# JuanTarrio/rebvo

Hardware: AMD Instinct MI355X
Metric: frames/sec (DoG+extract+track+depth) 752x480 EuRoC (higher is better)
Workload: dtype f32 scale-space / f64 tracker+EKF

## Files before the change

### rebvo_amd/csrc/api.hip

```cpp

#include <math.h>
#include <stdio.h>
#include <stdlib.h>
#include <string.h>

#include <algorithm>
#include <mutex>

#include "ctx.h"
#include "stage_a_dev.h"

namespace edgehip {

static thread_local std::string g_err;

int wait_pinned_ring(edgehip_ctx *c) {
    const int r = c->frames_seen % 8;
    if (c->ring_valid[r]) EH_CHECK(hipEventSynchronize(c->ev_ring[r]));
    return 0;
}

static int wait_idx_row(edgehip_ctx *c, int slot, const int32_t *pi) {
    if (c->slot_src[slot].idx_row != pi) return 0;
    if (c->a_api_valid[slot]) EH_CHECK(hipEventSynchronize(c->ev_a[slot]));
// ... 405 lines not shown
    }
    EH_TRY(dmalloc(c, &c->div_lut, kDivLutMax, al->dev));
    EH_TRY(dmalloc(c, &c->pinv, 3 * 49, al->dev, 0));
    EH_TRY(dmalloc(c, &c->seq, B, al->dev, 0));
    EH_TRY(dmalloc(c, &c->seqa, B, al->dev, 0));
    EH_TRY(dmalloc(c, &c->tresh_slot, S * B, al->dev, 0));
    c->fc_rows = std::max<int>(nslots, kRefRing);
    c->fc_index = 0;
    EH_TRY(dmalloc(c, &c->framecount, (size_t)c->fc_rows * B, al->dev, 0));
    EH_TRY(dmalloc(c, &c->kn_slot, S * B, al->dev, 0));
    EH_TRY(dmalloc(c, &c->retuned_slot, S * B, al->dev, 0));
    c->band_rows = detect_band_rows(p.w, p.plane_fit_size);
    c->nbands = (p.h - 2 * p.plane_fit_size + c->band_rows - 1) / c->band_rows;
    {
        const int npx = c->band_rows * p.w, nchunk = (npx + 63) / 64, cpw = (nchunk + kDetWaves - 1) / kDetWaves;
        c->band_cap = cpw * 64;
    }
    const size_t nstrips = (size_t)c->nbands * kDetWaves;
    EH_TRY(dmalloc(c, &c->band_cnt, B * nstrips, al->dev, 0));
    EH_TRY(dmalloc(c, &c->band_off, B * (nstrips + 1), al->dev, 0));
    {
        char *bs;
        EH_TRY(dmalloc(c, &bs, B * nstrips * c->band_cap * 20, al->dev));
        c->band_stage = bs;
    }
    EH_TRY(dmalloc(c, &c->histo, B * 256, al->dev, 0));
    c->nblk_tvr = (int)((CAP + kTvrBlock - 1) / kTvrBlock);
    EH_TRY(dmalloc(c, &c->P0, B * 3 * CAP, al->dev, 0));
    EH_TRY(dmalloc(c, &c->resid, (size_t)kResidBufs * B * CAP, al->dev, 0));
    EH_TRY(dmalloc(c, &c->resid_carry, (size_t)kResidBufs * B * c->nblk_tvr, al->dev, 0));
    EH_TRY(dmalloc(c, &c->partials, 2 * B * c->nblk_tvr * kNumSums, al->dev, 0));
    EH_TRY(dmalloc(c, &c->block_last, 2 * B * c->nblk_tvr, al->dev, 0));
    EH_TRY(dmalloc(c, &c->bin_cnt, B * 256, al->dev, 0));
    {
        const size_t ntiles = (size_t)((p.w + 63) / 64) * ((p.h + 63) / 64);
        EH_TRY(dmalloc(c, &c->bins, B * ntiles * CAP, al->dev));
    }
    c->field_radius = p.search_range;
    c->field_mode = EH_EXP_ENV("EDGEHIP_FIELD_MODE", 0);
    c->no_grec = getenv("EDGEHIP_NO_GREC") && atoi(getenv("EDGEHIP_NO_GREC")) != 0;
    c->level_mode = getenv("EDGEHIP_LEVEL_MODE") ? atoi(getenv("EDGEHIP_LEVEL_MODE")) : 0;
    c->fwd_mode = EH_EXP_ENV("EDGEHIP_FWD_MODE", 0);
    c->fused_min_batch = fused_min_env;
    c->fused_undist = EH_EXP_ENV("EDGEHIP_FUSED_UNDIST", 0) != 0;
    c->tvr_rw2 = EH_EXP_ENV("EDGEHIP_TVR_RW2", 0);
    c->dual_init = getenv("EDGEHIP_DUAL_INIT") ? atoi(getenv("EDGEHIP_DUAL_INIT")) : 1;
    c->persist_lm_max = EH_EXP_ENV("EDGEHIP_PERSIST_LM", 0);
    EH_TRY(dmalloc(c, &c->sync_cnt, B, al->dev, 0));
    EH_TRY(dmalloc(c, &c->fwd_key, B * CAP, al->dev, 0));
    EH_TRY(dmalloc(c, &c->fwd_win, B * CAP, al->dev, 0xFF));
    EH_TRY(dmalloc(c, &c->rs_tmp, B * 2 * CAP, al->dev, 0));
    c->fuse_match = !(getenv("EDGEHIP_FUSE_MATCH") && atoi(getenv("EDGEHIP_FUSE_MATCH")) == 0);
    if (c->fuse_match) {
        EH_TRY(dmalloc(c, &c->rot_pm, S * B * CAP, al->dev, 0)); EH_TRY(dmalloc(c, &c->rot_mm, S * B * CAP, al->dev, 0));
        EH_TRY(dmalloc(c, &c->rot_rho, S * B * CAP, al->dev, 0)); EH_TRY(dmalloc(c, &c->rot_srho, S * B * CAP, al->dev, 0));
    }
    EH_TRY(dmalloc(c, &c->rot_buf, B * 9, al->dev, 0));
    EH_TRY(dmalloc(c, &c->nav_dev, B, al->dev, 0));
    EH_TRY(dmalloc(c, &c->idx_dev, B, al->dev, 0));
    c->slot_src.assign(S, edgehip_ctx::SlotSrc());
    c->stereo_cnt = nullptr;
    if (p.stereo_available) EH_TRY(dmalloc(c, &c->stereo_cnt, B, al->dev, 0));
    c->nav_log = nullptr;
    c->nav_log_len = 0;

    {
        const size_t al256 = 256;
        auto up = [&](size_t x) { return (x + al256 - 1) / al256 * al256; };
        const bool stereo = p.stereo_available != 0;
        const size_t per = up(CAP * 4) * 8  +
                           up(CAP * 8) * 6  + up(CAP * 8) * 7  + up(CAP * 32) + up(CAP * 16)  +
                           (stereo ? up(CAP * 4) + 2 * up(CAP * 8) : 0);
        char *arena;
        EH_TRY(dmalloc(c, &arena, per * S * B, al->dev, 0));
        c->kl_arena = arena;
        c->kl.resize(S * B);
        for (size_t sb = 0; sb < S * B; sb++) {
            char *q = arena + sb * per;
            KlSoA &k = c->kl[sb];
            auto take = [&](size_t bytes) { char *r = q; q += up(bytes); return r; };
            k.p_inx = (int32_t *)take(CAP * 4);
            k.m_m = (float2 *)take(CAP * 8); k.u_m = (float2 *)take(CAP * 8); k.c_p = (float2 *)take(CAP * 8);
            k.p_m = (float2 *)take(CAP * 8); k.p_m_0 = (float2 *)take(CAP * 8); k.m_m0 = (float2 *)take(CAP * 8);
            k.n_m = (float *)take(CAP * 4);
            k.rho = (double *)take(CAP * 8); k.s_rho = (double *)take(CAP * 8); k.rho_nr = (double *)take(CAP * 8);
            k.s_rho_nr = (double *)take(CAP * 8); k.rho0 = (double *)take(CAP * 8); k.s_rho0 = (double *)take(CAP * 8);
            k.n_m0 = (double *)take(CAP * 8);
            k.m_id = (int32_t *)take(CAP * 4); k.m_id_f = (int32_t *)take(CAP * 4); k.m_id_kf = (int32_t *)take(CAP * 4);
            k.m_num = (int32_t *)take(CAP * 4); k.p_id = (int32_t *)take(CAP * 4); k.n_id = (int32_t *)take(CAP * 4);
            k.rec = (MatchRec *)take(CAP * 32);
            k.grec = (float4 *)take(CAP * 16);
            k.stereo_m_id = nullptr; k.stereo_rho = nullptr; k.stereo_s_rho = nullptr;
            if (stereo) {
                k.stereo_m_id = (int32_t *)take(CAP * 4);
                k.stereo_rho = (double *)take(CAP * 8); k.stereo_s_rho = (double *)take(CAP * 8);
            }
        }
        c->slot_cam.assign(S, edgehip_ctx::SlotCam{pl.ppx, pl.ppy, pl.zfm});
        EH_TRY(dmalloc(c, &c->kl_dev, S * B, al->dev));
        EH_CHECK(hipMemcpyAsync(c->kl_dev, c->kl.data(), sizeof(KlSoA) * S * B, hipMemcpyHostToDevice, c->stream));
    }
    {
        std::vector<float> lut(kDivLutMax, 0.f);
        for (int k = 1; k < kDivLutMax; k++) lut[k] = (float)(1.0 / (double)(float)k);
        EH_CHECK(hipMemcpyAsync(c->div_lut, lut.data(), sizeof(float) * kDivLutMax, hipMemcpyHostToDevice, c->stream));
        double pinv[3 * 49] = {0};
        plane_fit_pinv(p.plane_fit_size, pinv);
        if (p.plane_fit_size == 2)
// ... 1006 lines not shown
```

### rebvo_amd/csrc/ctx.h

```cpp
#pragma once
#include <hip/hip_runtime.h>
#include <stdint.h>
#include <string.h>
#include <string>
#include <map>
#include <vector>
#include <mutex>
#include <atomic>

#include "edgehip.h"
#include "export_ring.h"

namespace edgehip {

constexpr int kMaxBoxes = 3;
constexpr int kBandRows = 12;
constexpr int kDetWaves = 16;
constexpr int kDivLutMax = 256;
constexpr int kTvrThreads = 256;
constexpr int kTvrPasses = 1;
constexpr int kTvrBlock = kTvrThreads * kTvrPasses;
constexpr int kNumSums = 28;
constexpr int kRefRing = 8;
constexpr int kResidBufs = 3;

__host__ __device__ inline uint64_t resid_carry_bits() { return 0x7FF8C0DEC0DEC0DEull; }

struct __attribute__((aligned(16))) MatchRec {
    float c_px, c_py, u_mx, u_my, m_mx, m_my, n_m, pad;
};

struct KlSoA {
    int32_t *p_inx;
    float2 *m_m, *u_m, *c_p, *p_m, *p_m_0, *m_m0;
    float *n_m;
    double *rho, *s_rho, *rho_nr, *s_rho_nr, *rho0, *s_rho0, *n_m0;
    int32_t *m_id, *m_id_f, *m_id_kf, *m_num, *p_id, *n_id;
    MatchRec *rec;
    float4 *grec;
    int32_t *stereo_m_id;
    double *stereo_rho, *stereo_s_rho;
};

struct SeqDev {
    edgehip_seq_state pub;
    int32_t kn_new;
    int32_t band_trunc;
    float nm_max, nm_min;
    double tresh_used;
    double X[6], Xnew[6], Xt[6], h[6];
    double JtJ[36], JtF[6], JtJnew[36], JtFnew[6];
    double F, Fnew, F0, Ft, F0t, u, v, ut, vt, gain;
    int32_t eff_steps, eff_steps_t, res_cur, res_new, res_t, lm_phase;
    int32_t kn_old, pad1;
    double s_rho_min_eval;
    double Rt[9], Vt[3], RM[4];
    int32_t nmatch_tmp, kf_tmp;
    double zX[6], zXnew[6], zh[6];
    double zJtJ[36], zJtF[6], zJtJnew[36], zJtFnew[6];
    double zF, zFnew, zF0, zu, zv, zgain;
    double zRt[9], zVt[3], zRM[4];
    int32_t z_eff_steps, z_pad;
    double mv_V[3], mv_Vnew[3], mv_h[3], mv_JtJ[9], mv_JtF[3], mv_JtJnew[9], mv_JtFnew[3], mv_RVel[9];
    double mv_F, mv_Fnew, mv_u, mv_v, mv_s_rho_min;
    float mv_min_mod; int32_t mv_pad;
    int32_t skip_match, skip_map;
    double t_cur;
    double V_track[3], W_track[3], PV_track[9], PW_track[9];
};

struct SeqA {
    double tresh;
    double tresh_used;
    int32_t l_kl_num;
    int32_t kn_new;
    int32_t band_trunc, pad0;
    float nm_max, nm_min;
    float retuned, pad1;
};

struct DevicePlan {
    int w, h, n, cap, nseq, nslots;
    int ftx;
// ... 271 lines not shown
    edgehip::KlSoA *kl_dev;
    edgehip::SeqDev *seq;
    edgehip::SeqA *seqa;
    double *tresh_slot;
    uint32_t *framecount;
    int fc_rows;
    int fc_index;
    int32_t *kn_slot;
    float *retuned_slot;
    int32_t *band_cnt;
    int32_t *band_off;
    void *band_stage;
    int nbands, band_cap;
    int band_rows;
    int32_t *histo;
    double *P0;
    double *resid;
    double *resid_carry;
    double *partials;
    double *block_last;
    bool use_graph;
    std::map<int, hipGraphExec_t> frame_graphs;
    struct StereoRig {
        bool enabled = false;
        int slot_pair = -1;
        double t[3], R[9], max_radius;
    } rig;
    int ring_slots;
    struct SlotSrc { const uint8_t *base = nullptr; std::vector<int32_t> host_idx; bool grey8 = false;
                     const int32_t *idx_row = nullptr; int idx_ring = 0; };
    uint8_t *grey8 = nullptr;
    uint8_t *pinned_grey8 = nullptr;
    std::vector<SlotSrc> slot_src;
    struct SlotCam { float ppx, ppy; double zfm; };
    std::vector<SlotCam> slot_cam;
    int field_radius;
    int field_mode;
    int level_mode;
    int fused_min_batch;
    double pinv_host[3 * 49];
    int32_t *bin_cnt;
    int32_t *bins;
    int nblk_tvr;
    bool fused_undist;
    int tvr_rw2;
    bool tracker_f32 = false;
    int dual_init;
    int persist_lm_max;
    unsigned *sync_cnt;
    unsigned long long *fwd_key;
    int32_t *fwd_win;
    int fwd_mode = 0;
    bool fuse_match = true;
    float2 *rot_pm = nullptr, *rot_mm = nullptr;
    double *rot_rho = nullptr, *rot_srho = nullptr;
    bool rot_pending[4] = {false, false, false, false};
    bool fwd_fill[4] = {false, false, false, false};
    bool fwd_cleared = false;
    bool fwd_keys_posted = false;
    bool fwd_key_in_tvr = false;
    double *rs_tmp;
    double *rot_buf;
    const double *t_src = nullptr;
    edgehip_keyline *aos_dev = nullptr;
    edgehip_keyline *aos_host = nullptr;
    int32_t *aos_req_dev = nullptr, *aos_req_host = nullptr;
    int aos_requests = 0;
    edgehip::ExportRing kl_ring;
    edgehip::ExportRing ros_ring;
    edgehip_nav *nav_dev;
    edgehip_nav *nav_log;
    edgehip_nav_imu *nav_imu_log = nullptr;
    int nav_log_len;
    int32_t *stereo_log = nullptr;
    hipStream_t stream_log = nullptr;
    hipEvent_t ev_log = nullptr;
    hipEvent_t ev_log_ring[8] = {};
    std::mutex log_mu;
    std::atomic<long long> frames_logged{0};
    long long log_first = 0, log_last = -1;
    int32_t *idx_dev;
    int32_t *stereo_cnt;
    uint8_t *pinned_rgb;
    size_t pinned_rgb_bytes;
    edgehip::SeqDev *pinned_seq;
    edgehip::SeqA *pinned_seqa;
    double *pinned_out;
    double *pinned_t;
    int32_t *pinned_idx;
    edgehip_nav *pinned_nav;
    edgehip::Profiler *prof;
    bool imu_enabled = false, imu_pending = false;
    bool imu_pinned_ok = false;
    edgehip_imu_params imu_params;
    edgehip_kf_request *kf_req_dev = nullptr;
    edgehip_kf_result *kf_res_dev = nullptr;
    void *imu_track = nullptr;
    void *imu_filter = nullptr;
    void *imu_snap = nullptr;
    hipStream_t stream_imu = nullptr;
    hipEvent_t ev_imu_snap[2], ev_imu_post[2];
    hipEvent_t ev_imu_mid[2];
    bool imu_post_valid[2] = {false, false};
    edgehip_imu_integrated *imu_in_dev = nullptr;
    edgehip_nav_imu *nav_imu_dev = nullptr;
    edgehip_imu_integrated *pinned_imu = nullptr;
    edgehip_nav_imu *pinned_nav_imu = nullptr;
    struct DepthFill;
// ... 163 lines not shown
```

### rebvo_amd/csrc/stage_c.hip

```cpp

#include <math.h>
#include <string.h>

#include <vector>

#include "ctx.h"
#include "wave_reduce.h"

namespace edgehip {

constexpr double kRhoMax = 20.0, kRhoMin = 1e-3, kRhoInit = 1.0;

__global__ __launch_bounds__(256) void k_fwd_key(const KlSoA *kl_old, const int32_t *__restrict__ kn_old,
                                                 const int32_t *__restrict__ kn_new, unsigned long long *__restrict__ key,
                                                 int cap) {
    const int seq = blockIdx.z, i = blockIdx.x * 256 + threadIdx.x;
    if (i >= kn_old[seq]) return;
    const int f = kl_old[seq].m_id_f[i];
    if (f < 0 || f >= kn_new[seq]) return;
    atomicMax(&key[(size_t)seq * cap + f], ord_bits(kl_old[seq].rho[i]));
}
__device__ inline void so3_exp_c(const double w[3], double R[9]);
__device__ inline void rot_from_state(SeqDev *sq, double *__restrict__ Rbuf_seq);
__device__ inline void glue_after_tracking(SeqDev *sq);
__global__ __launch_bounds__(256) void k_fwd_win(const KlSoA *kl_old, const int32_t *__restrict__ kn_old,
                                                 const int32_t *__restrict__ kn_new, const unsigned long long *__restrict__ key,
                                                 int32_t *__restrict__ win, int cap, SeqDev *tail_seqs, double *__restrict__ tail_Rbuf) {
    const int seq = blockIdx.z, i = blockIdx.x * 256 + threadIdx.x;
    if (tail_seqs && i == 0) {
        rot_from_state(tail_seqs + seq, tail_Rbuf + (size_t)seq * 9);
        glue_after_tracking(tail_seqs + seq);
    }
    if (i >= kn_old[seq]) return;
    const int f = kl_old[seq].m_id_f[i];
    if (f < 0 || f >= kn_new[seq]) return;
    if (key[(size_t)seq * cap + f] == ord_bits(kl_old[seq].rho[i])) atomicMax(&win[(size_t)seq * cap + f], i);
}
template <bool FILL>
__global__ __launch_bounds__(256) void k_fwd_apply(const KlSoA *kl_old, const KlSoA *kl_new, const int32_t *__restrict__ kn_new,
                                                   const int32_t *__restrict__ win, SeqDev *seqs, int cap) {
    const int seq = blockIdx.z, f = blockIdx.x * 256 + threadIdx.x;
    int hit = 0;
    if (f < kn_new[seq]) {
        const int i = win[(size_t)seq * cap + f];
        const KlSoA &o = kl_old[seq], &n = kl_new[seq];
        if (i >= 0 || FILL) {
            double rho = kRhoInit, s_rho = kRhoMax, rho_nr = kRhoInit, s_rho_nr = kRhoMax;
            int32_t m_num = -1, m_id_kf = -1;
            float2 pm = make_float2(0.f, 0.f), mm = make_float2(0.f, 0.f);
            float nm = 0.f;
            if (i >= 0) {
                rho = o.rho[i]; s_rho = o.s_rho[i]; rho_nr = o.rho_nr[i]; s_rho_nr = o.s_rho_nr[i];
                m_num = o.m_num[i]; m_id_kf = o.m_id_kf[i];
                pm = o.p_m[i]; mm = o.m_m[i];
                nm = o.n_m[i];
            } else {
                pm = n.p_m[f];
            }
            n.rho[f] = rho;
            n.s_rho[f] = s_rho;
            n.rho_nr[f] = rho_nr;
            n.s_rho_nr[f] = s_rho_nr;
            n.m_num[f] = m_num + 1;
            n.m_id[f] = i;
            n.p_m_0[f] = pm;
            n.m_m0[f] = mm;
            n.n_m0[f] = (double)nm;
            n.m_id_kf[f] = m_id_kf;
            hit = i >= 0;
        }
    }
    const int cnt = __popcll(__ballot(hit));
    if ((threadIdx.x & 63) == 0 && cnt) atomicAdd(&seqs[seq].pub.klm_fwd, cnt);
}

__device__ inline void so3_exp_c(const double w[3], double R[9]);

struct RotOut {
    float2 *p_m, *m_m;
    double *rho, *s_rho;
};
struct WinArgs {
    const int32_t *kn_new;
    const unsigned long long *key;
    int32_t *win;
    SeqDev *seqs;
    double *Rbuf;
};
template <bool OUT, bool WIN>
__global__ __launch_bounds__(256) void k_rotate(const KlSoA *kls, const int32_t *__restrict__ kns, const double *__restrict__ Rin,
                                                double zf, RotOut out, int cap, WinArgs wa) {
    const int seq = blockIdx.z, i = blockIdx.x * 256 + threadIdx.x;
    __shared__ double s_R[9];
    if (WIN) {
        if (blockIdx.x * 256 >= kns[seq] && blockIdx.x != 0) return;
        if (threadIdx.x == 0) {
            SeqDev *sq = wa.seqs + seq;
            double R0[9];
            so3_exp_c(sq->pub.W, R0);
            for (int q = 0; q < 9; q++) s_R[q] = R0[q];
            if (blockIdx.x == 0) {
                for (int q = 0; q < 9; q++) wa.Rbuf[(size_t)seq * 9 + q] = R0[q];
                for (int a = 0; a < 3; a++)
                    for (int b = 0; b < 3; b++) sq->pub.R[a * 3 + b] = R0[b * 3 + a];
                glue_after_tracking(sq);
            }
        }
        __syncthreads();
    }
    if (i >= kns[seq]) return;
    double Rw[9];
    if (WIN) {
#pragma unroll
        for (int q = 0; q < 9; q++) {
            const double v = s_R[q];
            const unsigned lo = __builtin_amdgcn_readfirstlane((unsigned)__double2loint(v)), hi = __builtin_amdgcn_readfirstlane((unsigned)__double2hiint(v));
            Rw[q] = __hiloint2double((int)hi, (int)lo);
        }
    }
    const double *R = WIN ? Rw : Rin + (size_t)seq * 9;
    const KlSoA &k = kls[seq];
    const float2 pm = k.p_m[i];
    const float2 m = k.m_m[i];
    const double rho = k.rho[i], s_rho = k.s_rho[i];
    const double v0 = (double)pm.x / zf, v1 = (double)pm.y / zf, v2 = 1;
    double q0 = 0, q1 = 0, q2 = 0;
    q0 += R[0] * v0; q0 += R[1] * v1; q0 += R[2] * v2;
    q1 += R[3] * v0; q1 += R[4] * v1; q1 += R[5] * v2;
    q2 += R[6] * v0; q2 += R[7] * v1; q2 += R[8] * v2;
    const double m0 = (double)m.x, m1 = (double)m.y;
    double r0 = 0, r1 = 0;
    r0 += R[0] * m0; r0 += R[1] * m1; r0 += R[2] * 0.0;
    r1 += R[3] * m0; r1 += R[4] * m1; r1 += R[5] * 0.0;
    const float2 mr = make_float2((float)r0, (float)r1);
    if (WIN) {
        const int f = k.m_id_f[i];
        if (f >= 0 && f < wa.kn_new[seq] && wa.key[(size_t)seq * cap + f] == ord_bits(rho)) atomicMax(&wa.win[(size_t)seq * cap + f], i);
    }
    if (OUT) {
        const size_t o = (size_t)seq * cap + i;
        const bool turn = fabs(q2) > 0;
#if EDGEHIP_NT_ROT
        st_stream(out.p_m + o, turn ? make_float2((float)(q0 / q2 * zf), (float)(q1 / q2 * zf)) : pm);
        st_stream(out.rho + o, turn ? rho / q2 : rho);
        st_stream(out.s_rho + o, turn ? s_rho / q2 : s_rho);
        st_stream(out.m_m + o, mr);
#else
        out.p_m[o] = turn ? make_float2((float)(q0 / q2 * zf), (float)(q1 / q2 * zf)) : pm;
        out.rho[o] = turn ? rho / q2 : rho;
        out.s_rho[o] = turn ? s_rho / q2 : s_rho;
        out.m_m[o] = mr;
#endif
        return;
    }
    if (fabs(q2) > 0) {
        k.p_m[i] = make_float2((float)(q0 / q2 * zf), (float)(q1 / q2 * zf));
        k.rho[i] = rho / q2;
        k.s_rho[i] = s_rho / q2;
    }
    k.m_m[i] = mr;
}

__global__ __launch_bounds__(256) void k_rot_materialize(const KlSoA *kls, const int32_t *__restrict__ kns, RotOut src, int cap) {
    const int seq = blockIdx.z, i = blockIdx.x * 256 + threadIdx.x;
    if (i >= kns[seq]) return;
    const KlSoA &k = kls[seq];
    const size_t o = (size_t)seq * cap + i;
    const float2 pm = src.p_m[o], mm = src.m_m[o];
    const double rho = src.rho[o], s_rho = src.s_rho[o];
    k.p_m[i] = pm; k.m_m[i] = mm; k.rho[i] = rho; k.s_rho[i] = s_rho;
}
static RotOut rot_of(edgehip_ctx *c, int slot) {
    const size_t off = (size_t)slot * c->plan.nseq * c->plan.cap;
    RotOut r;
    r.p_m = c->rot_pm + off; r.m_m = c->rot_mm + off; r.rho = c->rot_rho + off; r.s_rho = c->rot_srho + off;
    return r;
}
int rot_materialize_enqueue(edgehip_ctx *c, int slot) {
    if (slot < 0 || slot >= c->plan.nslots || !c->rot_pending[slot]) return 0;
    const DevicePlan &pl = c->plan;
    hipLaunchKernelGGL(k_rot_materialize, dim3((pl.cap + 255) / 256, 1, pl.nseq), dim3(256), 0, c->stream, kldev(c, slot),
                       c->kn_slot + (size_t)slot * pl.nseq, rot_of(c, slot), pl.cap);
    EH_LAUNCH_CHECK();
    c->rot_pending[slot] = false;
    return 0;
}

__global__ __launch_bounds__(256) void k_rec_refresh(const KlSoA *kls, const int32_t *__restrict__ kns) {
    const int seq = blockIdx.z, i = blockIdx.x * 256 + threadIdx.x;
    if (i >= kns[seq]) return;
    const KlSoA &k = kls[seq];
    const float2 cp = k.c_p[i], um = k.u_m[i], m = k.m_m[i];
    const float nm = k.n_m[i];
    MatchRec rec;
    rec.c_px = cp.x; rec.c_py = cp.y; rec.u_mx = um.x; rec.u_my = um.y;
    rec.m_mx = m.x; rec.m_my = m.y; rec.n_m = nm; rec.pad = 0.f;
    k.rec[i] = rec;
}
int rec_refresh_enqueue(edgehip_ctx *c, int slot) {
    if (int e = rot_materialize_enqueue(c, slot)) return e;
    if (!c->rec_stale[slot]) return 0;
    const DevicePlan &pl = c->plan;
    hipLaunchKernelGGL(k_rec_refresh, dim3((pl.cap + 255) / 256, 1, pl.nseq), dim3(256), 0, c->stream, kldev(c, slot),
                       c->kn_slot + (size_t)slot * pl.nseq);
    EH_LAUNCH_CHECK();
    c->rec_stale[slot] = false;
    return 0;
}

#ifdef EDGEHIP_EXPERIMENTS
__global__ __launch_bounds__(256) void k_fwd_apply_rotate(const KlSoA *kl_old, const KlSoA *kl_new, const int32_t *__restrict__ kn_old,
                                                          const int32_t *__restrict__ kn_new, const int32_t *__restrict__ win,
                                                          SeqDev *seqs, const double *__restrict__ Rin, double zf, int cap) {
    const int seq = blockIdx.z, i = blockIdx.x * 256 + threadIdx.x;
    int hit = 0;
    if (i < kn_old[seq]) {
        const KlSoA &o = kl_old[seq];
        const int f = o.m_id_f[i];
        const float2 pm = o.p_m[i];
        const float2 m = o.m_m[i];
        const double rho = o.rho[i], s_rho = o.s_rho[i];
        if (f >= 0 && f < kn_new[seq] && win[(size_t)seq * cap + f] == i) {
            const KlSoA &n = kl_new[seq];
            const double rho_nr = o.rho_nr[i], s_rho_nr = o.s_rho_nr[i];
            const int32_t m_num = o.m_num[i], m_id_kf = o.m_id_kf[i];
            const float nm = o.n_m[i];
            n.rho[f] = rho;
            n.s_rho[f] = s_rho;
// ... 53 lines not shown
    r[0] = (M[7] - M[5]) / 2;
    r[1] = (M[2] - M[6]) / 2;
    r[2] = (M[3] - M[1]) / 2;
    const double sin_angle_abs = sqrt(r[0] * r[0] + r[1] * r[1] + r[2] * r[2]);
    if (cos_angle > M_SQRT1_2) {
        if (sin_angle_abs > 0) {
            const double s = asin(sin_angle_abs) / sin_angle_abs;
            r[0] *= s; r[1] *= s; r[2] *= s;
        }
    } else if (cos_angle > -M_SQRT1_2) {
        const double s = acos(cos_angle) / sin_angle_abs;
        r[0] *= s; r[1] *= s; r[2] *= s;
    } else {
        const double angle = M_PI - asin(sin_angle_abs);
        const double d0 = M[0] - cos_angle, d1 = M[4] - cos_angle, d2 = M[8] - cos_angle;
        double r2[3];
        if (d0 * d0 > d1 * d1 && d0 * d0 > d2 * d2) { r2[0] = d0; r2[1] = (M[3] + M[1]) / 2; r2[2] = (M[2] + M[6]) / 2; }
        else if (d1 * d1 > d2 * d2) { r2[0] = (M[3] + M[1]) / 2; r2[1] = d1; r2[2] = (M[7] + M[5]) / 2; }
        else { r2[0] = (M[2] + M[6]) / 2; r2[1] = (M[7] + M[5]) / 2; r2[2] = d2; }
        if (r2[0] * r[0] + r2[1] * r[1] + r2[2] * r[2] < 0) { r2[0] = -r2[0]; r2[1] = -r2[1]; r2[2] = -r2[2]; }
        const double nn = sqrt(r2[0] * r2[0] + r2[1] * r2[1] + r2[2] * r2[2]);
        for (int i = 0; i < 3; i++) r[i] = angle * (r2[i] / nn);
    }
}

__device__ inline void rot_from_state(SeqDev *sq, double *__restrict__ Rbuf_seq) {
    double R0[9];
    so3_exp_c(sq->pub.W, R0);
    for (int i = 0; i < 9; i++) Rbuf_seq[i] = R0[i];
    for (int i = 0; i < 3; i++)
        for (int j = 0; j < 3; j++) sq->pub.R[i * 3 + j] = R0[j * 3 + i];
}
__global__ void k_rot_from_state(SeqDev *seqs, double *__restrict__ Rbuf, int nseq) {
    const int seq = blockIdx.x * blockDim.x + threadIdx.x;
    if (seq >= nseq) return;
    rot_from_state(seqs + seq, Rbuf + (size_t)seq * 9);
}

struct DirArgs {
    const KlSoA *kl_new, *kl_old;
    const int32_t *kn_new;
    const int32_t *mask_old;
    SeqDev *seq;
    int w, h;
    size_t n;
    double zfm, min_thr_mod, cang_min_edge, max_radius, loc_unc;
    float ppx, ppy;
    int stereo_mode;
    const int32_t *win;
    RotOut rot;
    int cap;
};

#ifndef EDGEHIP_NT_ROT
#define EDGEHIP_NT_ROT 1
#endif
#ifndef EDGEHIP_NT_EKF
#define EDGEHIP_NT_EKF 1
#endif
#ifndef EDGEHIP_NT_DIRECTED
#define EDGEHIP_NT_DIRECTED 1
#endif
template <bool FUSED, bool FILL>
__device__ __forceinline__ void directed_body(const DirArgs &a) {
    const int seq = blockIdx.z, ik = blockIdx.x * (int)blockDim.x + threadIdx.x;
    SeqDev *sq = a.seq + seq;
    const bool searching = !sq->skip_match;
    if (!FUSED && !searching) return;
    __shared__ double s_v[3], s_rv[9], s_br[9];
    if (threadIdx.x == 0 && searching) {
        const double *BR = sq->pub.R, *V = sq->pub.V, *P = sq->pub.P_V;
        for (int i = 0; i < 9; i++) s_br[i] = BR[i];
        for (int i = 0; i < 3; i++) {
            double d = 0;
            for (int j = 0; j < 3; j++) d += BR[i * 3 + j] * V[j];
            s_v[i] = d;
        }
        double T[9];
        for (int i = 0; i < 3; i++)
            for (int j = 0; j < 3; j++) {
                double d = 0;
                for (int k = 0; k < 3; k++) d += BR[i * 3 + k] * P[k * 3 + j];
                T[i * 3 + j] = d;
            }
        for (int i = 0; i < 3; i++)
            for (int j = 0; j < 3; j++) {
                double d = 0;
                for (int k = 0; k < 3; k++) d += T[i * 3 + k] * BR[j * 3 + k];
                s_rv[i * 3 + j] = d;
            }
    }
    __syncthreads();
    int matched = 0, kfm = 0, fwd = 0;
    if (ik < a.kn_new[seq]) {
        const KlSoA &kn = a.kl_new[seq], &ko = a.kl_old[seq];
        const int32_t *mask = a.mask_old + (size_t)seq * a.n;
        const size_t ro = (size_t)seq * a.cap;
        const float2 kpm = ldg(kn.p_m, ik);
        const float2 kmm = ldg(kn.m_m, ik);
        const float knm = ldg(kn.n_m, ik);
        int iw = -1;
        double krho, ksrho;
        if (FUSED) {
            iw = a.win[ro + ik];
            fwd = iw >= 0;
            if (iw >= 0) { krho = ldg(ko.rho, iw); ksrho = ldg(ko.s_rho, iw); }
            else if (FILL) { krho = kRhoInit; ksrho = kRhoMax; }
            else { krho = ldg(kn.rho, ik); ksrho = ldg(kn.s_rho, ik); }
        } else {
            krho = ldg(kn.rho, ik); ksrho = ldg(kn.s_rho, ik);
        }
        int found = -1;
        if (searching) {
        const double zf = a.zfm;
        double p3[3];
        for (int i = 0; i < 3; i++) {
            double d = 0;
            d += s_br[i * 3 + 0] * (double)kpm.x;
// ... 47 lines not shown
            dq_rho = 0;
            t_steps = (int)dq_max;
        }
        const double norm_m = (double)knm;
        constexpr int DM_CH = 2;
        const double Tmax = (double)(a.w + a.h) + fabs((double)pi0x) + fabs((double)pi0y) + 4.0;
        int seg0[2] = {0, 0}, seg1[2] = {t_steps, 0};
        int nseg = 1;
        if (t_steps > 256 && fabs(dq_rho) < 1e15 && Tmax < 1e15) {
            const double n0 = fmax(0.0, floor(dq_rho - Tmax) - 2.0), n1 = fmin((double)t_steps, ceil(fmin(dq_rho + Tmax, dq_rho - dq_min)) + 2.0);
            const double p0 = fmax(0.0, floor(-Tmax - dq_rho - 1.0) - 2.0), p1 = fmin((double)t_steps, ceil(fmin(Tmax - dq_rho - 1.0, dq_max - dq_rho - 1.0)) + 2.0);
            const bool hn = n1 > n0, hp = p1 > p0;
            nseg = 0;
            if (hn && hp && !(n1 < p0 || p1 < n0)) {
                seg0[0] = (int)fmin(n0, p0); seg1[0] = (int)fmax(n1, p1); nseg = 1;
            } else {
                if (hn) { seg0[nseg] = (int)n0; seg1[nseg] = (int)n1; nseg++; }
                if (hp) { seg0[nseg] = (int)p0; seg1[nseg] = (int)p1; nseg++; }
                if (nseg == 2 && seg0[1] < seg0[0]) {
                    const int s0 = seg0[0], s1 = seg1[0];
                    seg0[0] = seg0[1]; seg1[0] = seg1[1]; seg0[1] = s0; seg1[1] = s1;
                }
            }
        }
        for (int sg = 0; sg < nseg && found < 0; sg++) {
        double tn = dq_rho - (double)seg0[sg], tp = (dq_rho + 1) + (double)seg0[sg];
        const int t_end = seg1[sg];
        for (int t0i = seg0[sg]; t0i < t_end && found < 0; t0i += DM_CH) {
            double tv[DM_CH][2];
            int jm[DM_CH][2];
#pragma unroll
            for (int c = 0; c < DM_CH; c++) {
                tv[c][0] = tn; tv[c][1] = tp;
                tn -= 1; tp += 1;
#pragma unroll
                for (int dir = 0; dir < 2; dir++) {
                    const double t = tv[c][dir];
                    jm[c][dir] = -1;
                    if (t0i + c >= t_end) continue;
                    if (dir ? t > dq_max : t < dq_min) continue;
                    const float fx = (float)(t_x * t + (double)pi0x), fy = (float)(t_y * t + (double)pi0y);
                    const int xi = round_half_away_i(fx), yi = round_half_away_i(fy);
                    if (xi >= a.w || yi >= a.h || xi < 0 || yi < 0) continue;
                    jm[c][dir] = mask[__umul24((unsigned)yi, (unsigned)a.w) + (unsigned)xi];
                }
            }
#pragma unroll
            for (int c = 0; c < DM_CH; c++) {
#pragma unroll
                for (int dir = 0; dir < 2; dir++) {
                    const int j = jm[c][dir];
                    if (j < 0 || found >= 0) continue;
                    const double t = tv[c][dir];
                    const float2 omm = FUSED ? ldg(a.rot.m_m, ro + j) : ldg(ko.m_m, j);
                    const double norm_m0 = (double)ldg(ko.n_m, j);
                    const double cang = div_mid((double)(omm.x * kmm.x + omm.y * kmm.y), norm_m0 * norm_m);
                    if (cang < a.cang_min_edge || fabs(norm_m0 / norm_m - 1) > a.min_thr_mod) continue;
                    const double s_rho = FUSED ? ldg(a.rot.s_rho, ro + j) : ldg(ko.s_rho, j), rho = FUSED ? ldg(a.rot.rho, ro + j) : ldg(ko.rho, j);
                    const double v_rho_dr = (a.loc_unc * a.loc_unc + s_rho * s_rho * norm_t * norm_t + sigma2_t * rho * rho);
                    const double dd = t - norm_t * rho;
                    if (dd * dd > v_rho_dr) continue;
                    found = j;
                }
            }
        }
        }
        }
        if (FUSED) {
            const int src = found >= 0 ? found : iw;
            if (src >= 0 || FILL) {
                double rho = kRhoInit, s_rho = kRhoMax, rho_nr = kRhoInit, s_rho_nr = kRhoMax;
                int32_t m_num = -1, m_id_kf = -1;
                float2 pm, mm = make_float2(0.f, 0.f);
                float nm = 0.f;
                if (src < 0) {
                    pm = ldg(kn.p_m, ik);
                } else {
                    const bool turned = found >= 0;
                    rho = turned ? ldg(a.rot.rho, ro + src) : ldg(ko.rho, src);
                    s_rho = turned ? ldg(a.rot.s_rho, ro + src) : ldg(ko.s_rho, src);
                    pm = turned ? ldg(a.rot.p_m, ro + src) : ldg(ko.p_m, src);
                    mm = turned ? ldg(a.rot.m_m, ro + src) : ldg(ko.m_m, src);
                    rho_nr = ldg(ko.rho_nr, src); s_rho_nr = ldg(ko.s_rho_nr, src);
                    m_num = ldg(ko.m_num, src); m_id_kf = ldg(ko.m_id_kf, src);
                    nm = ldg(ko.n_m, src);
                }
#if EDGEHIP_NT_DIRECTED
                stg_stream(kn.rho, ik, rho);
                stg_stream(kn.s_rho, ik, s_rho);
                stg_stream(kn.rho_nr, ik, rho_nr);
                stg_stream(kn.s_rho_nr, ik, s_rho_nr);
                stg_stream(kn.m_num, ik, m_num + 1);
                stg_stream(kn.m_id, ik, src);
                stg_stream(kn.p_m_0, ik, pm);
                stg_stream(kn.m_m0, ik, mm);
                stg_stream(kn.n_m0, ik, (double)nm);
                stg_stream(kn.m_id_kf, ik, m_id_kf);
#else
                stg(kn.rho, ik, rho);
                stg(kn.s_rho, ik, s_rho);
                stg(kn.rho_nr, ik, rho_nr);
                stg(kn.s_rho_nr, ik, s_rho_nr);
                stg(kn.m_num, ik, m_num + 1);
                stg(kn.m_id, ik, src);
                stg(kn.p_m_0, ik, pm);
                stg(kn.m_m0, ik, mm);
                stg(kn.n_m0, ik, (double)nm);
                stg(kn.m_id_kf, ik, m_id_kf);
#endif
                matched = found >= 0;
                kfm = matched && m_id_kf >= 0;
            }
        } else if (found >= 0) {
            const int j = found;
            const double c_rho = a.stereo_mode ? ldg(ko.rho0, j) : ldg(ko.rho, j), c_srho = a.stereo_mode ? ldg(ko.s_rho0, j) : ldg(ko.s_rho, j);
            double c_rho_nr = 0, c_srho_nr = 0;
            if (!a.stereo_mode) { c_rho_nr = ldg(ko.rho_nr, j); c_srho_nr = ldg(ko.s_rho_nr, j); }
            const int32_t c_mnum = ldg(ko.m_num, j), mk = ldg(ko.m_id_kf, j);
            const float2 c_pm = ldg(ko.p_m, j), c_mm = ldg(ko.m_m, j);
            const float c_nm = ldg(ko.n_m, j);
            stg(kn.rho, ik, c_rho);
            stg(kn.s_rho, ik, c_srho);
            if (!a.stereo_mode) {
                stg(kn.rho_nr, ik, c_rho_nr);
                stg(kn.s_rho_nr, ik, c_srho_nr);
            }
            stg(kn.m_id, ik, j);
            stg(kn.m_num, ik, c_mnum + 1);
            stg(kn.p_m_0, ik, c_pm);
            stg(kn.m_m0, ik, c_mm);
            stg(kn.n_m0, ik, (double)c_nm);
            stg(kn.m_id_kf, ik, mk);
            matched = 1;
            kfm = mk >= 0;
        }
    }
    const int c1 = __popcll(__ballot(matched)), c2 = __popcll(__ballot(kfm)), c3 = FUSED ? __popcll(__ballot(fwd)) : 0;
    if ((threadIdx.x & 63) == 0) {
// ... 496 lines not shown
        if (!c->fwd_cleared) EH_CHECK(hipMemsetAsync(c->fwd_win, 0xFF, sizeof(int32_t) * B * pl.cap, c->stream));
        c->fwd_cleared = false;
        hipLaunchKernelGGL(k_fwd_win, g, b, 0, c->stream, kldev(c, slot_old), kno, knn, c->fwd_key, c->fwd_win, pl.cap,
                           (SeqDev *)nullptr, (double *)nullptr);
        hipLaunchKernelGGL(k_rot_from_state, dim3((pl.nseq + 63) / 64), dim3(64), 0, c->stream, c->seq, c->rot_buf, pl.nseq);
        EH_LAUNCH_CHECK();
    }
    ProfScope ps(c, PROF_C_ROTATE);
    hipLaunchKernelGGL(k_fwd_apply_rotate, g, b, 0, c->stream, kldev(c, slot_old), kldev(c, slot_new), kno, knn, c->fwd_win, c->seq,
                       c->rot_buf, pl.zfm, pl.cap);
    EH_LAUNCH_CHECK();
    return 0;
}
#endif

static inline bool frame_matches_in_one_pass(const edgehip_ctx *c, int slot_pair) {
    return c->fuse_match && c->fwd_mode == 0 && slot_pair < 0 && !c->p.stereo_available;
}

static int forward_rotate_one_pass_enqueue(edgehip_ctx *c, int slot_old, int slot_new) {
    if (int e = rot_materialize_enqueue(c, slot_old)) return e;
    const DevicePlan &pl = c->plan;
    const size_t B = pl.nseq;
    const bool cleared = c->fwd_cleared;
    c->fwd_cleared = false;
    if (!cleared) EH_CHECK(hipMemsetAsync(c->fwd_win, 0xFF, sizeof(int32_t) * B * pl.cap, c->stream));
    c->grec_ok[slot_old] = false;
    c->rec_stale[slot_old] = true;
    ProfScope ps(c, PROF_C_ROTATE);
    WinArgs wa;
    wa.kn_new = c->kn_slot + slot_new * B; wa.key = c->fwd_key; wa.win = c->fwd_win; wa.seqs = c->seq; wa.Rbuf = c->rot_buf;
    hipLaunchKernelGGL((k_rotate<true, true>), dim3((pl.cap + 255) / 256, 1, pl.nseq), dim3(256), 0, c->stream, kldev(c, slot_old),
                       c->kn_slot + slot_old * B, (const double *)nullptr, pl.zfm, rot_of(c, slot_old), pl.cap, wa);
    EH_LAUNCH_CHECK();
    c->rot_pending[slot_old] = true;
    return 0;
}

int rotate_enqueue(edgehip_ctx *c, int slot, const double *R_host, bool R_in_buf) {
    if (int e = rot_materialize_enqueue(c, slot)) return e;
    c->grec_ok[slot] = false;
    c->rec_stale[slot] = true;
    ProfScope ps(c, PROF_C_ROTATE);
    const DevicePlan &pl = c->plan;
    double *Rbuf = c->rot_buf;
    if (R_host) {
        EH_CHECK(hipStreamSynchronize(c->stream));
        memcpy(c->pinned_out, R_host, sizeof(double) * 9 * pl.nseq);
        EH_CHECK(hipMemcpyAsync(Rbuf, c->pinned_out, sizeof(double) * 9 * pl.nseq, hipMemcpyHostToDevice, c->stream));
    } else if (!R_in_buf) {
        hipLaunchKernelGGL(k_rot_from_state, dim3((pl.nseq + 63) / 64), dim3(64), 0, c->stream, c->seq, Rbuf, pl.nseq);
    }
    hipLaunchKernelGGL((k_rotate<false, false>), dim3((pl.cap + 255) / 256, 1, pl.nseq), dim3(256), 0, c->stream, kldev(c, slot),
                       c->kn_slot + (size_t)slot * pl.nseq, Rbuf, pl.zfm, RotOut{nullptr, nullptr, nullptr, nullptr}, pl.cap, WinArgs{});
    EH_LAUNCH_CHECK();
    return 0;
}

struct StereoArgs {
    const KlSoA *kl, *kl_pair;
    const int32_t *kn;
    const int32_t *mask_pair;
    int32_t *nmatch;
    int w, h;
    size_t n;
    double t[3], R[9];
    double zfm0, zfm1;
    float pp1x, pp1y;
    double min_thr_mod, cang_min_edge, max_radius, loc_unc, loc_unc_model;
    const SeqDev *seqs;
};

__global__ __launch_bounds__(256) void k_stereo_match(StereoArgs a) {
    const int seq = blockIdx.z, i = blockIdx.x * 256 + threadIdx.x;
    if (a.seqs && a.seqs[seq].skip_map) return;
    int matched = 0;
    if (i < a.kn[seq]) {
        const KlSoA &k = a.kl[seq], &kp = a.kl_pair[seq];
        const int32_t *mask = a.mask_pair + (size_t)seq * a.n;
        const float2 pm = k.p_m[i], mm = k.m_m[i];
        const float nm = k.n_m[i];
        const double rho = k.rho[i], s_rho = k.s_rho[i];
        const double lo = rho - s_rho, hi = rho + s_rho;
        const double min_rho = lo < 1e-3 ? 1e-3 : lo, max_rho = 20.0 < hi ? 20.0 : hi;
        double q1[2][3];
#pragma unroll
        for (int e = 0; e < 2; e++) {
            const double r = e ? max_rho : min_rho;
            const double p0[3] = {(double)pm.x / r / a.zfm0, (double)pm.y / r / a.zfm0, 1.0 / r};
            double p1[3];
#pragma unroll
            for (int c = 0; c < 3; c++) {
                double d = 0;
                d += a.R[c * 3 + 0] * p0[0]; d += a.R[c * 3 + 1] * p0[1]; d += a.R[c * 3 + 2] * p0[2];
                p1[c] = d + a.t[c];
            }
            q1[e][0] = p1[0] / p1[2] * a.zfm1; q1[e][1] = p1[1] / p1[2] * a.zfm1; q1[e][2] = 1 / p1[2];
        }
        const double dqx = q1[1][0] - q1[0][0], dqy = q1[1][1] - q1[0][1];
        const double pi0x = q1[0][0] + (double)a.pp1x, pi0y = q1[0][1] + (double)a.pp1y;
        double norm_t = sqrt(dqx * dqx + dqy * dqy);
        double t_x, t_y, dq_min, dq_max;
        if (norm_t > 1e-6) {
            t_x = dqx / norm_t;
            t_y = dqy / norm_t;
            dq_min = -a.loc_unc;
            dq_max = fmin(a.max_radius, norm_t + a.loc_unc);
// ... 47 lines not shown
            const double mul = (double)(-u.x) * (zf1 * qh1[0] - qx * qh1[2]) - uy * (zf1 * qh1[1] - qy * qh1[2]);
            double srho = mul / div;
            const double den = qh1[2] + a.t[2] * srho;
            const double df = ux * zf1 * (a.t[0] * den - a.t[2] * (qh1[0] + a.t[0] * srho)) / (den * den) +
                              uy * zf1 * (a.t[1] * den - a.t[2] * (qh1[1] + a.t[1] * srho)) / (den * den);
            double I_rho = (df / a.loc_unc_model) * (df / a.loc_unc_model);
            if (srho != srho || df != df) { srho = 1; I_rho = 1e-10; }
            double ss = 1 / sqrt(I_rho);
            if (srho < 0) { ss = 1e3; srho = 1.0; match = -1; }
            k.stereo_rho[i] = srho;
            k.stereo_s_rho[i] = ss;
        }
        k.stereo_m_id[i] = match;
        matched = match >= 0;
    }
    const int c1 = __popcll(__ballot(matched));
    if ((threadIdx.x & 63) == 0 && c1) atomicAdd(&a.nmatch[seq], c1);
}

__global__ __launch_bounds__(256) void k_fuse_stereo(const KlSoA *kls, const int32_t *__restrict__ kns, SeqDev *seqs) {
    const int seq = blockIdx.z, i = blockIdx.x * 256 + threadIdx.x;
    if (seqs) {
        if (seqs[seq].skip_map) return;
        if (i == 0) seqs[seq].pub.Kp = 1;
    }
    if (i >= kns[seq]) return;
    const KlSoA &k = kls[seq];
    const double r0 = k.rho[i], s0 = k.s_rho[i];
    k.rho0[i] = r0;
    k.s_rho0[i] = s0;
    if (k.stereo_m_id[i] < 0) return;
    const double sr = k.stereo_rho[i], ss = k.stereo_s_rho[i];
    const double s = sqrt(1.0 / (1.0 / (s0 * s0) + 1.0 / (ss * ss)));
    k.s_rho[i] = s;
    k.rho[i] = (r0 / (s0 * s0) + sr / (ss * ss)) * (s * s);
}

int directed_enqueue(edgehip_ctx *c, int slot_new, int slot_old, bool fused) {
    ProfScope ps(c, PROF_C_DIRECTED);
    const DevicePlan &pl = c->plan;
    if (!fused) { if (int e = rot_materialize_enqueue(c, slot_old)) return e; }
    DirArgs a;
    a.kl_new = kldev(c, slot_new); a.kl_old = kldev(c, slot_old);
    a.kn_new = c->kn_slot + (size_t)slot_new * pl.nseq;
    a.mask_old = maskof(c, slot_old);
    a.seq = c->seq; a.w = pl.w; a.h = pl.h; a.n = pl.n; a.zfm = pl.zfm;
    a.min_thr_mod = c->p.match_thresh_module;
    a.cang_min_edge = cos(c->p.match_thresh_angle * M_PI / 180.0);
    a.max_radius = (double)c->p.search_range;
    a.loc_unc = c->p.loc_unc_match;
    a.ppx = pl.ppx; a.ppy = pl.ppy;
    a.stereo_mode = c->p.stereo_available != 0;
    a.win = c->fwd_win; a.cap = pl.cap;
    a.rot = fused ? rot_of(c, slot_old) : RotOut{nullptr, nullptr, nullptr, nullptr};
#ifndef EDGEHIP_DIRECTED_BLOCK
#define EDGEHIP_DIRECTED_BLOCK 128
#endif
    constexpr int kDirBlock = EDGEHIP_DIRECTED_BLOCK;
    const dim3 g((pl.cap + kDirBlock - 1) / kDirBlock, 1, pl.nseq), b(kDirBlock);
    if (fused) {
        if (c->fwd_fill[slot_new]) hipLaunchKernelGGL(k_directed_fused<true>, g, b, 0, c->stream, a);
        else hipLaunchKernelGGL(k_directed_fused<false>, g, b, 0, c->stream, a);
        c->fwd_fill[slot_new] = false;
    } else {
        hipLaunchKernelGGL(k_directed, g, b, 0, c->stream, a);
    }
    EH_LAUNCH_CHECK();
    return 0;
}

int regekf_enqueue(edgehip_ctx *c, int slot, int do_reg, int do_ekf, bool frame_glue) {
    ProfScope ps(c, PROF_C_REGEKF);
    const DevicePlan &pl = c->plan;
    dim3 g((pl.cap + 255) / 256, 1, pl.nseq), b(256);
    const int32_t *kn = c->kn_slot + (size_t)slot * pl.nseq;
    hipLaunchKernelGGL(k_regularize, g, b, 0, c->stream, kldev(c, slot), kn, c->rs_tmp, c->seq, pl.cap,
                       c->p.regularize_thresh, do_reg, frame_glue ? c->p.global_match_threshold : -1);
    hipLaunchKernelGGL(k_ekf, g, b, 0, c->stream, kldev(c, slot), kn, c->rs_tmp, c->seq, pl.cap, pl.zfm, c->p.reshape_q_abs,
                       c->p.loc_unc, do_ekf);
    EH_LAUNCH_CHECK();
    return 0;
}

int rescale_enqueue(edgehip_ctx *c, int slot, bool frame_ends) {
    ProfScope ps(c, PROF_C_RESCALE);
    const DevicePlan &pl = c->plan;
    FrameEndArgs fe = {};
    if (frame_ends) {
        fe.nav = c->nav_dev;
        fe.kn_new = c->kn_slot + (size_t)slot * pl.nseq;
        const int slot_t = c->rig.enabled && c->rig.slot_pair >= 0 ? c->rig.slot_pair : slot;
        fe.tresh_new = c->tresh_slot + (size_t)slot_t * pl.nseq;
        fe.retuned_new = c->retuned_slot + (size_t)slot * pl.nseq;
        fe.nav_log = c->nav_log; fe.nav_log_len = c->nav_log_len; fe.nseq = pl.nseq; fe.have_pair = 1;
    }
    if (!c->lds_optin_rescale) {
        EH_CHECK(hipFuncSetAttribute((const void *)&k_rescale<512, 12, 4>, hipFuncAttributeMaxDynamicSharedMemorySize, 4 * 4 * 1024 * (int)sizeof(double)));
        c->lds_optin_rescale = true;
    }
    hipLaunchKernelGGL((k_rescale<512, 12, 4>), dim3(pl.nseq), dim3(512), 4 * 4 * 1024 * sizeof(double), c->stream, kldev(c, slot),
                       c->kn_slot + (size_t)slot * pl.nseq, c->seq, kRhoMax, 1u, c->p.do_rescaling > 0, fe);
    EH_LAUNCH_CHECK();
    return 0;
}

static int rotate_buf_enqueue(edgehip_ctx *c, int slot) {
    if (int e = rot_materialize_enqueue(c, slot)) return e;
    c->grec_ok[slot] = false;
    c->rec_stale[slot] = true;
    ProfScope ps(c, PROF_C_ROTATE);
    const DevicePlan &pl = c->plan;
    hipLaunchKernelGGL((k_rotate<false, false>), dim3((pl.cap + 255) / 256, 1, pl.nseq), dim3(256), 0, c->stream, kldev(c, slot),
                       c->kn_slot + (size_t)slot * pl.nseq, c->rot_buf, pl.zfm, RotOut{nullptr, nullptr, nullptr, nullptr}, pl.cap, WinArgs{});
    EH_LAUNCH_CHECK();
    return 0;
}
static int ext_rotvel_enqueue(edgehip_ctx *c, int slot) {
    const DevicePlan &pl = c->plan;
    const int B = pl.nseq, nblk = (pl.cap + 255) / 256;
    if (nblk > c->nblk_tvr) { set_error("ext_rot_vel: partial table too small"); return EDGEHIP_ERR_STATE; }
    hipLaunchKernelGGL(k_ext_rotvel, dim3(nblk, 1, B), dim3(256), 0, c->stream, kldev(c, slot), c->kn_slot + (size_t)slot * B,
                       (const double *)nullptr, c->seq, c->partials, c->nblk_tvr, pl.zfm, c->p.loc_unc, c->p.reweight_distance);
    EH_LAUNCH_CHECK();
    return 0;
}

static int glue(edgehip_ctx *c, int mode, int slot_new, int have_pair) {
    const DevicePlan &pl = c->plan;
    const int slot_t = c->rig.enabled && c->rig.slot_pair >= 0 ? c->rig.slot_pair : slot_new;
    hipLaunchKernelGGL(k_frame_glue, dim3((pl.nseq + 63) / 64), dim3(64), 0, c->stream, c->seq, c->t_src, c->nav_dev,
                       c->kn_slot + (size_t)slot_new * pl.nseq, c->tresh_slot + (size_t)slot_t * pl.nseq,
                       c->retuned_slot + (size_t)slot_new * pl.nseq, pl.nseq, mode, c->p.config_fps, c->p.global_match_threshold,
                       have_pair, c->nav_log, c->nav_log_len, c->stereo_cnt, c->rig.enabled ? c->stereo_log : nullptr);
    EH_LAUNCH_CHECK();
    return 0;
}

}

using namespace edgehip;

extern "C" {

static int chk2(edgehip_ctx *c, int a, int b) {
    if (!c || a < 0 || b < 0 || a >= c->plan.nslots || b >= c->plan.nslots) { set_error("slot out of range"); return EDGEHIP_ERR_ARG; }
    if (int e = rot_materialize_enqueue(c, a)) return e;
    return rot_materialize_enqueue(c, b);
}

int edgehip_forward_match(edgehip_ctx *c, int slot_old, int slot_new) {
    EH_ENTER(c);
    if (int e = chk2(c, slot_old, slot_new)) return e;
    return forward_match_enqueue(c, slot_old, slot_new);
}
int edgehip_rotate_keylines(edgehip_ctx *c, int slot, const double *R) {
    EH_ENTER(c);
    if (int e = chk2(c, slot, slot)) return e;
    return rotate_enqueue(c, slot, R);
}
int edgehip_directed_matching(edgehip_ctx *c, int slot_new, int slot_old) {
    EH_ENTER(c);
    if (int e = chk2(c, slot_new, slot_old)) return e;
    return directed_enqueue(c, slot_new, slot_old);
}
int edgehip_match_one_pass(edgehip_ctx *c, int slot_new, int slot_old, int fill) {
    EH_ENTER(c);
// ... 404 lines not shown
```

Measured before the change: 135,500.

## Pack rotated keyline fields into a 32-byte record for the fused matcher

Replaces the separate rotated-buffer arrays for m_m, rho and s_rho with one 32-byte RotRec per keyline that also carries n_m. The rotate kernel writes it with vector nontemporal stores, and the fused directed matcher reads it with two vector loads. The goal is fewer scattered memory transactions on the random-access match candidates. It also adds an XCD-contiguous block remapping for the fused directed kernel, which is off by default.

```diff
diff --git a/rebvo_amd/csrc/api.hip b/rebvo_amd/csrc/api.hip
--- a/rebvo_amd/csrc/api.hip
+++ b/rebvo_amd/csrc/api.hip
@@ -481,8 +481,7 @@
     EH_TRY(dmalloc(c, &c->rs_tmp, B * 2 * CAP, al->dev, 0));
     c->fuse_match = !(getenv("EDGEHIP_FUSE_MATCH") && atoi(getenv("EDGEHIP_FUSE_MATCH")) == 0);
     if (c->fuse_match) {
-        EH_TRY(dmalloc(c, &c->rot_pm, S * B * CAP, al->dev, 0)); EH_TRY(dmalloc(c, &c->rot_mm, S * B * CAP, al->dev, 0));
-        EH_TRY(dmalloc(c, &c->rot_rho, S * B * CAP, al->dev, 0)); EH_TRY(dmalloc(c, &c->rot_srho, S * B * CAP, al->dev, 0));
+        EH_TRY(dmalloc(c, &c->rot_pm, S * B * CAP, al->dev, 0)); EH_TRY(dmalloc(c, &c->rot_rec, S * B * CAP, al->dev, 0));
     }
     EH_TRY(dmalloc(c, &c->rot_buf, B * 9, al->dev, 0));
     EH_TRY(dmalloc(c, &c->nav_dev, B, al->dev, 0));
diff --git a/rebvo_amd/csrc/ctx.h b/rebvo_amd/csrc/ctx.h
--- a/rebvo_amd/csrc/ctx.h
+++ b/rebvo_amd/csrc/ctx.h
@@ -10,6 +10,7 @@
 
 #include "edgehip.h"
 #include "export_ring.h"
+#include "xcd_order.h"
 
 namespace edgehip {
 
@@ -29,6 +30,12 @@
 struct __attribute__((aligned(16))) MatchRec {
     float c_px, c_py, u_mx, u_my, m_mx, m_my, n_m, pad;
 };
+
+struct __attribute__((aligned(32))) RotRec {
+    double rho, s_rho;
+    float m_mx, m_my, n_m, pad;
+};
+static_assert(sizeof(RotRec) == 32, "two RotRec per 64-byte line");
 
 struct KlSoA {
     int32_t *p_inx;
@@ -406,8 +413,8 @@
     int32_t *fwd_win;
     int fwd_mode = 0;
     bool fuse_match = true;
-    float2 *rot_pm = nullptr, *rot_mm = nullptr;
-    double *rot_rho = nullptr, *rot_srho = nullptr;
+    float2 *rot_pm = nullptr;
+    edgehip::RotRec *rot_rec = nullptr;
     bool rot_pending[4] = {false, false, false, false};
     bool fwd_fill[4] = {false, false, false, false};
     bool fwd_cleared = false;
diff --git a/rebvo_amd/csrc/stage_c.hip b/rebvo_amd/csrc/stage_c.hip
--- a/rebvo_amd/csrc/stage_c.hip
+++ b/rebvo_amd/csrc/stage_c.hip
@@ -10,6 +10,10 @@
 namespace edgehip {
 
 constexpr double kRhoMax = 20.0, kRhoMin = 1e-3, kRhoInit = 1.0;
+
+#ifndef EDGEHIP_NT_ROT
+#define EDGEHIP_NT_ROT 1
+#endif
 
 __global__ __launch_bounds__(256) void k_fwd_key(const KlSoA *kl_old, const int32_t *__restrict__ kn_old,
                                                  const int32_t *__restrict__ kn_new, unsigned long long *__restrict__ key,
@@ -77,9 +81,27 @@
 __device__ inline void so3_exp_c(const double w[3], double R[9]);
 
 struct RotOut {
-    float2 *p_m, *m_m;
-    double *rho, *s_rho;
+    float2 *p_m;
+    RotRec *rec;
 };
+typedef double rot_d2 __attribute__((ext_vector_type(2)));
+typedef float rot_f4 __attribute__((ext_vector_type(4)));
+__device__ __forceinline__ void rotrec_store(RotRec *p, double rho, double s_rho, float2 mm, float nm) {
+#if EDGEHIP_NT_ROT
+    __builtin_nontemporal_store(rot_d2{rho, s_rho}, reinterpret_cast<rot_d2 *>(p));
+    __builtin_nontemporal_store(rot_f4{mm.x, mm.y, nm, 0.f}, reinterpret_cast<rot_f4 *>(p) + 1);
+#else
+    *reinterpret_cast<rot_d2 *>(p) = rot_d2{rho, s_rho};
+    *(reinterpret_cast<rot_f4 *>(p) + 1) = rot_f4{mm.x, mm.y, nm, 0.f};
+#endif
+}
+__device__ __forceinline__ void rotrec_load(const RotRec *p, size_t i, double &rho, double &s_rho, float2 &mm, float &nm) {
+    typedef const rot_d2 __attribute__((address_space(1))) GD;
+    typedef const rot_f4 __attribute__((address_space(1))) GF;
+    const rot_d2 a = *(GD *)(p + i);
+    const rot_f4 b = *((GF *)(p + i) + 1);
+    rho = a.x; s_rho = a.y; mm = make_float2(b.x, b.y); nm = b.z;
+}
 struct WinArgs {
     const int32_t *kn_new;
     const unsigned long long *key;
@@ -123,6 +145,8 @@
     const float2 pm = k.p_m[i];
     const float2 m = k.m_m[i];
     const double rho = k.rho[i], s_rho = k.s_rho[i];
+    float nm = 0.f;
+    if (OUT) nm = k.n_m[i];
     const double v0 = (double)pm.x / zf, v1 = (double)pm.y / zf, v2 = 1;
     double q0 = 0, q1 = 0, q2 = 0;
     q0 += R[0] * v0; q0 += R[1] * v1; q0 += R[2] * v2;
@@ -142,15 +166,10 @@
         const bool turn = fabs(q2) > 0;
 #if EDGEHIP_NT_ROT
         st_stream(out.p_m + o, turn ? make_float2((float)(q0 / q2 * zf), (float)(q1 / q2 * zf)) : pm);
-        st_stream(out.rho + o, turn ? rho / q2 : rho);
-        st_stream(out.s_rho + o, turn ? s_rho / q2 : s_rho);
-        st_stream(out.m_m + o, mr);
 #else
         out.p_m[o] = turn ? make_float2((float)(q0 / q2 * zf), (float)(q1 / q2 * zf)) : pm;
-        out.rho[o] = turn ? rho / q2 : rho;
-        out.s_rho[o] = turn ? s_rho / q2 : s_rho;
-        out.m_m[o] = mr;
 #endif
+        rotrec_store(out.rec + o, turn ? rho / q2 : rho, turn ? s_rho / q2 : s_rho, mr, nm);
         return;
     }
     if (fabs(q2) > 0) {
@@ -166,14 +185,17 @@
     if (i >= kns[seq]) return;
     const KlSoA &k = kls[seq];
     const size_t o = (size_t)seq * cap + i;
-    const float2 pm = src.p_m[o], mm = src.m_m[o];
-    const double rho = src.rho[o], s_rho = src.s_rho[o];
+    const float2 pm = src.p_m[o];
+    float2 mm;
+    double rho, s_rho;
+    float nm;
+    rotrec_load(src.rec, o, rho, s_rho, mm, nm);
     k.p_m[i] = pm; k.m_m[i] = mm; k.rho[i] = rho; k.s_rho[i] = s_rho;
 }
 static RotOut rot_of(edgehip_ctx *c, int slot) {
     const size_t off = (size_t)slot * c->plan.nseq * c->plan.cap;
     RotOut r;
-    r.p_m = c->rot_pm + off; r.m_m = c->rot_mm + off; r.rho = c->rot_rho + off; r.s_rho = c->rot_srho + off;
+    r.p_m = c->rot_pm + off; r.rec = c->rot_rec + off;
     return r;
 }
 int rot_materialize_enqueue(edgehip_ctx *c, int slot) {
@@ -333,9 +355,6 @@
     int cap;
 };
 
-#ifndef EDGEHIP_NT_ROT
-#define EDGEHIP_NT_ROT 1
-#endif
 #ifndef EDGEHIP_NT_EKF
 #define EDGEHIP_NT_EKF 1
 #endif
@@ -344,7 +363,16 @@
 #endif
 template <bool FUSED, bool FILL>
 __device__ __forceinline__ void directed_body(const DirArgs &a) {
-    const int seq = blockIdx.z, ik = blockIdx.x * (int)blockDim.x + threadIdx.x;
+#ifndef EDGEHIP_DIRECTED_XCD
+#define EDGEHIP_DIRECTED_XCD 0
+#endif
+    const int seq = blockIdx.z;
+    int bx = (int)blockIdx.x;
+    if (FUSED && EDGEHIP_DIRECTED_XCD) {
+        const int nb = (a.kn_new[seq] + (int)blockDim.x - 1) / (int)blockDim.x;
+        if (bx < nb) bx = xcd_contiguous(bx, nb);
+    }
+    const int ik = bx * (int)blockDim.x + threadIdx.x;
     SeqDev *sq = a.seq + seq;
     const bool searching = !sq->skip_match;
     if (!FUSED && !searching) return;
@@ -498,11 +526,19 @@
                     const int j = jm[c][dir];
                     if (j < 0 || found >= 0) continue;
                     const double t = tv[c][dir];
-                    const float2 omm = FUSED ? ldg(a.rot.m_m, ro + j) : ldg(ko.m_m, j);
-                    const double norm_m0 = (double)ldg(ko.n_m, j);
+                    float2 omm;
+                    float onm;
+                    double s_rho = 0, rho = 0;
+                    if (FUSED) {
+                        rotrec_load(a.rot.rec, ro + j, rho, s_rho, omm, onm);
+                    } else {
+                        omm = ldg(ko.m_m, j);
+                        onm = ldg(ko.n_m, j);
+                    }
+                    const double norm_m0 = (double)onm;
                     const double cang = div_mid((double)(omm.x * kmm.x + omm.y * kmm.y), norm_m0 * norm_m);
                     if (cang < a.cang_min_edge || fabs(norm_m0 / norm_m - 1) > a.min_thr_mod) continue;
-                    const double s_rho = FUSED ? ldg(a.rot.s_rho, ro + j) : ldg(ko.s_rho, j), rho = FUSED ? ldg(a.rot.rho, ro + j) : ldg(ko.rho, j);
+                    if (!FUSED) { s_rho = ldg(ko.s_rho, j); rho = ldg(ko.rho, j); }
                     const double v_rho_dr = (a.loc_unc * a.loc_unc + s_rho * s_rho * norm_t * norm_t + sigma2_t * rho * rho);
                     const double dd = t - norm_t * rho;
                     if (dd * dd > v_rho_dr) continue;
@@ -523,13 +559,16 @@
                     pm = ldg(kn.p_m, ik);
                 } else {
                     const bool turned = found >= 0;
-                    rho = turned ? ldg(a.rot.rho, ro + src) : ldg(ko.rho, src);
-                    s_rho = turned ? ldg(a.rot.s_rho, ro + src) : ldg(ko.s_rho, src);
-                    pm = turned ? ldg(a.rot.p_m, ro + src) : ldg(ko.p_m, src);
-                    mm = turned ? ldg(a.rot.m_m, ro + src) : ldg(ko.m_m, src);
+                    if (turned) {
+                        rotrec_load(a.rot.rec, ro + src, rho, s_rho, mm, nm);
+                        pm = ldg(a.rot.p_m, ro + src);
+                    } else {
+                        rho = ldg(ko.rho, src); s_rho = ldg(ko.s_rho, src);
+                        pm = ldg(ko.p_m, src); mm = ldg(ko.m_m, src);
+                        nm = ldg(ko.n_m, src);
+                    }
                     rho_nr = ldg(ko.rho_nr, src); s_rho_nr = ldg(ko.s_rho_nr, src);
                     m_num = ldg(ko.m_num, src); m_id_kf = ldg(ko.m_id_kf, src);
-                    nm = ldg(ko.n_m, src);
                 }
 #if EDGEHIP_NT_DIRECTED
                 stg_stream(kn.rho, ik, rho);
@@ -1132,7 +1171,7 @@
         hipLaunchKernelGGL(k_rot_from_state, dim3((pl.nseq + 63) / 64), dim3(64), 0, c->stream, c->seq, Rbuf, pl.nseq);
     }
     hipLaunchKernelGGL((k_rotate<false, false>), dim3((pl.cap + 255) / 256, 1, pl.nseq), dim3(256), 0, c->stream, kldev(c, slot),
-                       c->kn_slot + (size_t)slot * pl.nseq, Rbuf, pl.zfm, RotOut{nullptr, nullptr, nullptr, nullptr}, pl.cap, WinArgs{});
+                       c->kn_slot + (size_t)slot * pl.nseq, Rbuf, pl.zfm, RotOut{nullptr, nullptr}, pl.cap, WinArgs{});
     EH_LAUNCH_CHECK();
     return 0;
 }
@@ -1286,7 +1325,7 @@
     a.ppx = pl.ppx; a.ppy = pl.ppy;
     a.stereo_mode = c->p.stereo_available != 0;
     a.win = c->fwd_win; a.cap = pl.cap;
-    a.rot = fused ? rot_of(c, slot_old) : RotOut{nullptr, nullptr, nullptr, nullptr};
+    a.rot = fused ? rot_of(c, slot_old) : RotOut{nullptr, nullptr};
 #ifndef EDGEHIP_DIRECTED_BLOCK
 #define EDGEHIP_DIRECTED_BLOCK 128
 #endif
@@ -1345,7 +1384,7 @@
     ProfScope ps(c, PROF_C_ROTATE);
     const DevicePlan &pl = c->plan;
     hipLaunchKernelGGL((k_rotate<false, false>), dim3((pl.cap + 255) / 256, 1, pl.nseq), dim3(256), 0, c->stream, kldev(c, slot),
-                       c->kn_slot + (size_t)slot * pl.nseq, c->rot_buf, pl.zfm, RotOut{nullptr, nullptr, nullptr, nullptr}, pl.cap, WinArgs{});
+                       c->kn_slot + (size_t)slot * pl.nseq, c->rot_buf, pl.zfm, RotOut{nullptr, nullptr}, pl.cap, WinArgs{});
     EH_LAUNCH_CHECK();
     return 0;
 }
diff --git a/rebvo_amd/csrc/xcd_order.h b/rebvo_amd/csrc/xcd_order.h
--- /dev/null
+++ b/rebvo_amd/csrc/xcd_order.h
@@ -0,0 +1,18 @@
+#pragma once
+
+#if defined(__HIPCC__) || defined(__CUDACC__)
+#define EDGEHIP_HD __host__ __device__
+#else
+#define EDGEHIP_HD
+#endif
+
+namespace edgehip {
+
+constexpr int kXcds = 8;
+
+EDGEHIP_HD constexpr int xcd_contiguous(int p, int n) {
+    const int q = n / kXcds, m = n % kXcds, r = p % kXcds;
+    return r * q + (r < m ? r : m) + p / kXcds;
+}
+
+}
```

Measured after the change: 133,900. 0.988x the previous value.
